# GATB/MindTheGap

Measured on AMD Instinct MI355X. Metric: breakpoints filled/sec, higher is better.
Workload: dtype u64; 1 GPU; synthetic human-scale: 3 Gbp i.i.d. donor as 600000 x 5 kb sequences, 100000 insertion sites (50-1000 nt) per batch, k=31, max-nodes 100; sites_per_batch=100000, sites_per_rank_and_step=100000, distinct_batches_per_rank=4, site_set=400000, donor_sequences=600000, erroneous_fragments=0, k=31, max_nodes=100, max_length=10000, nb_solid_kmers=3108581096, nb_unitigs=600024, index_bytes=60154587216, unitig_store_bytes=3945966160, batches_in_flight=6, input=prepared batches, resident in HBM, output=C-ABI records + ASCII sequences in page-locked host memory

## Files before the change

mindthegap_amd/csrc/mtg_emit.h:

```cpp
#ifndef MTG_EMIT_H
#define MTG_EMIT_H
#include "../../include/mtg_fill.h"
#include "mtg_copy.h"

namespace mtg {

enum : uint8_t { GAPF_REPEATED = 1, GAPF_REVERSE = 2 };

MTG_DEV void emit_plan(const GapOut& o, const PostOut& p, bool want_all, int k, uint32_t& nw, uint32_t& nc, uint32_t& asc, uint32_t& ext)
{
    nw = nc = asc = ext = 0;
    if (o.status != GAP_OK) return;
    if (want_all || (p.fast == 0 && p.nb_terminal > 0)) { nw = o.n_words; nc = o.n_contigs; }
    if (want_all) return;
    if (p.fast == 1) asc = p.pos - (uint32_t)k + 1u;
    else if (p.nb_terminal == 0 && o.n_contigs > 0 && p.clen0 > (uint32_t)k) ext = p.clen0 - (uint32_t)k + 1u;
}

struct PartTot {
    uint64_t begin[4], end[4];
    uint64_t lines, store_runs, run_nt, contig_nt, contig_words, post_lines, cov_kmers, copy_words, copy_cmds, cov_direct, n_lean;
    uint64_t copy_words_exec, copy_cmds_exec, scan_words;
    uint32_t n_retry, n_general, n_filled, n_ext;
    uint32_t n_parked, n_branching;
// ... 68 lines not shown
            U64x2 v;
            v.x = (uint64_t)out[0] | ((uint64_t)out[1] << 32);
            v.y = (uint64_t)out[2] | ((uint64_t)out[3] << 32);
            *reinterpret_cast<U64x2*>(d) = v;
        } else {
            for (uint32_t b = 0; b < n; b++) d[b] = (char)((out[b >> 2] >> (8u * (b & 3u))) & 0xFFu);
        }
    }
    if (lane == 0 && !(pk.half && aoff + L >= pk.x)) dst[L] = 0;
}
MTG_DEV void emit_ascii(const uint64_t* src, uint32_t from, uint32_t L, bool rc, char* dst) { emit_ascii_g<MTG_NLANES>(src, from, L, rc, dst, MTG_LANE()); }

struct EmitHost {
    char* seq;
    char* ext;
    mtg_filled* fil;
};
struct EmitDev {
    char* seq;
    char* ext;
    uint64_t seq_cap, ext_cap;
    mtg_gap_result* res;
    mtg_filled* fil;
    uint64_t* dense_words;
    uint32_t* dense_meta;
    uint64_t dense_cap_words, dense_cap_contigs;
    uint8_t* wire;
    uint64_t wire_cap, wire_tag;
    const PartTot* tot;
    uint32_t wire_gaps;
    uint32_t* shadow = nullptr;
    uint64_t shadow_cap = 0;
    uint32_t pack_q = 0;
};
MTG_DEV PackedTail packed_tail(const EmitDev& D) { return PackedTail{D.shadow, D.shadow ? packed_split(D.tot->end[2], D.pack_q) : 0ull, D.shadow_cap}; }
struct WireLayout {
    uint64_t o_gaps, o_filled, o_seq, o_ext, total;
};
MTG_HD WireLayout wire_layout(uint64_t n_gaps, uint64_t n_filled, uint64_t seq_bytes, uint64_t ext_bytes)
{
    WireLayout w;
    w.o_gaps = sizeof(mtg_wire_header);
    w.o_filled = w.o_gaps + ((n_gaps * sizeof(mtg_wire_gap) + 7) & ~7ull);
    w.o_seq = w.o_filled + ((n_filled * sizeof(mtg_wire_filled) + 7) & ~7ull);
    w.o_ext = w.o_seq + ((seq_bytes + 7) & ~7ull);
    w.total = w.o_ext + ((ext_bytes + 7) & ~7ull);
    return w;
}
MTG_HD uint64_t wire_word_sum(uint64_t w, uint64_t i) { return (w ^ (i * 0x9E3779B97F4A7C15ull)) * 0xBF58476D1CE4E5B9ull; }

MTG_DEV int qual_of(uint32_t errors, bool repeated)
{
    int q = repeated ? 25 : 50;
    if (errors == 1) q = 10;
    if (errors == 2) q = 5;
    return q;
}

MTG_DEV mtg_filled filled_of(const PostOut& p, uint64_t abase, uint32_t flags, const EmitHost& H)
{
    mtg_filled f;
    f.seq = H.seq + abase;
    f.nb_errors_in_anchor = (int)p.errors;
    f.target_index = (int)p.target;
#ifdef MTG_EMU
    f.avg_coverage = (float)p.ab_sum / (float)p.ab_n;
// ... 124 lines not shown
```

mindthegap_amd/csrc/mtg_gpu_fill.hip:

```cpp
#include "mtg_gpu_common.h"

namespace mtgi {

enum { TRAVERSAL_SETS = mtg_index::NWS };
__constant__ Index c_ix[TRAVERSAL_SETS];
__constant__ FillCfg c_cfg[TRAVERSAL_SETS];

#ifndef MTG_STAGE_A_WAVES
#define MTG_STAGE_A_WAVES 2
#endif
#ifndef MTG_WALK_WAVES
#define MTG_WALK_WAVES 2
#endif
enum { PARK_LISTS = 19 };
struct ParkCtl {
    uint32_t count[PARK_LISTS];
    uint32_t n_branching;
    uint32_t pad_[3];
#ifdef MTG_BUBBLE_TIMING
    uint32_t hist_lane[32], hist_wave[32], hist_walk_lane[32], hist_walk_wave[32];
#endif
};
#ifdef MTG_BUBBLE_TIMING
__device__ __forceinline__ void timing_note(uint32_t* hl, uint32_t* hw, uint64_t t0)
// ... 447 lines not shown
    for (uint32_t li = blockIdx.x; li < count; li += gridDim.x) {
    const uint32_t slot = use_list ? park_list(park, n, POST_LIST)[li] : li;
    __syncthreads();
    if (threadIdx.x == 0) {
        r = recs[slot];
        const ScanBlock& b = blocks[slot / SCAN_SL];
        r.wbase += b.v[0]; r.cbase += b.v[1]; r.abase += b.v[2]; r.ebase += b.v[3];
        r.rpos += (uint32_t)b.v[4]; r.gpos += (uint32_t)b.v[5]; r.fpos += (uint32_t)b.v[6];
        recs[slot] = r;
        if (r.o.status != GAP_OK) retry_list[r.rpos] = slot;
        else if (r.nc) general_list[r.gpos] = slot;
    }
    __syncthreads();
    GapScratch S;
    S.z = nullptr;
    S.v = nullptr;
    S.lane = slot & 63u;
    S.r = raw + (uint64_t)slot * cfg.raw_stride;
    S.h = head + (uint64_t)(slot >> 6) * cfg.hd_stride;
    const uint32_t g = ids ? ids[slot] : slot;
    emit_gap(us, cfg, S, r, gflags[g], slot, g, k, D, H);
    }
}
#ifndef MTG_EMIT_LEAN_G
#define MTG_EMIT_LEAN_G 8
#endif
enum { EMIT_LEAN_G = MTG_EMIT_LEAN_G };
__global__ void __launch_bounds__(64) k_emit_lean(UStore us, FillCfg cfg, uint8_t* raw, uint8_t* head, const SlotRec* __restrict__ recs, const ScanBlock* __restrict__ blocks, const uint32_t* __restrict__ ids,
                                                  const uint8_t* __restrict__ gflags, int k, EmitDev D, EmitHost H, uint32_t n)
{
    const uint32_t slot = blockIdx.x * (64u / EMIT_LEAN_G) + threadIdx.x / EMIT_LEAN_G, gl = threadIdx.x % EMIT_LEAN_G;
    if (slot >= n) return;
    const SlotRec r = recs[slot];
    if (!emit_is_lean(r, D)) return;
    GapScratch S;
    S.z = nullptr;
    S.v = nullptr;
    S.lane = slot & 63u;
    S.r = raw + (uint64_t)slot * cfg.raw_stride;
    S.h = head + (uint64_t)(slot >> 6) * cfg.hd_stride;
    const uint32_t g = ids ? ids[slot] : slot;
    emit_lean<EMIT_LEAN_G>(us, cfg, S, r, r.abase + blocks[slot / SCAN_SL].v[2], gflags[g], slot, g, k, D, H, gl);
}

__global__ void __launch_bounds__(256) k_wire_sum(uint8_t* wire, uint64_t cap)
{
    mtg_wire_header* h = reinterpret_cast<mtg_wire_header*>(wire);
    if (h->magic != 0x3145524957474D54ull || h->total_bytes > cap) return;
    const uint64_t* w = reinterpret_cast<const uint64_t*>(wire + sizeof(mtg_wire_header));
    const uint64_t n = (h->total_bytes - sizeof(mtg_wire_header)) / 8;
    uint64_t s = 0;
    for (uint64_t i = (uint64_t)blockIdx.x * blockDim.x + threadIdx.x; i < n; i += (uint64_t)gridDim.x * blockDim.x) s += wire_word_sum(w[i], i);
    for (int d = 32; d >= 1; d >>= 1) {
        const uint32_t lo = (uint32_t)__shfl_xor((int)(uint32_t)s, d, 64), hi = (uint32_t)__shfl_xor((int)(uint32_t)(s >> 32), d, 64);
        s += ((uint64_t)hi << 32) | lo;
    }
    if ((threadIdx.x & 63u) == 0 && s) atomicAdd(reinterpret_cast<unsigned long long*>(&h->checksum), (unsigned long long)s);
}

__global__ void __launch_bounds__(64) k_paths(FillCfg cfg, uint8_t* raw, uint8_t* head, const GapOut* __restrict__ outs, const uint32_t* __restrict__ slots, int k, uint32_t* out, uint32_t n)
{
    __shared__ PathsWork W;
    if (blockIdx.x >= n) return;
    const uint32_t slot = slots[blockIdx.x];
    GapScratch S;
    S.z = nullptr;
    S.v = nullptr;
    S.lane = slot & 63u;
    S.r = raw + (uint64_t)slot * cfg.raw_stride;
    S.h = head + (uint64_t)(slot >> 6) * cfg.hd_stride;
    paths_gap(cfg, S, outs[slot], k, W, out + (uint64_t)blockIdx.x * PATHS_WORDS);
}

__global__ void __launch_bounds__(64) k_general(Index ix, FillCfg cfg, uint8_t* raw, uint8_t* head, const GapOut* __restrict__ outs, const uint32_t* __restrict__ slots, const uint32_t* __restrict__ ids,
                                                const uint32_t* __restrict__ paths, const uint32_t* __restrict__ tcnt, const uint8_t* __restrict__ fast_ok, const uint64_t* __restrict__ src,
// ... 228 lines not shown
    uint64_t* d_tbad = d_tle + n_targets;
    uint32_t* d_pi_head = nullptr;
    uint32_t* d_pi_next = nullptr;
    uint32_t pi_mask = 0;
    uint8_t* d_tie_p = nullptr;
    if (seeds) {
        d_pi_head = const_cast<uint32_t*>(in.shared.pi);
        d_pi_next = d_pi_head + (size_t)in.shared.pi_mask + 1;
        pi_mask = in.shared.pi_mask;
        HIP_TRY(d_tie.alloc(n));
        d_tie_p = d_tie.as<uint8_t>();
        HIP_TRY(hipMemsetAsync(d_tie_p, 0, n, stream));
    } else if (n_targets >= (uint64_t)POST_INDEX_MIN * n && n_targets < (1ull << 30) && !tune::on(tune::T_NO_POST_INDEX)) {
        uint64_t cap = 1024;
        while (cap < 4 * n_targets) cap <<= 1;
        HIP_TRY(d_pidx.alloc((cap + 4 * n_targets) * 4));
        d_pi_head = d_pidx.as<uint32_t>();
        d_pi_next = d_pi_head + cap;
        pi_mask = (uint32_t)(cap - 1);
        HIP_TRY(hipMemsetAsync(d_pi_head, 0xFF, cap * 4, stream));
        hipLaunchKernelGGL(k_post_index, dim3((unsigned)std::min<size_t>(n, 4096)), dim3(256), 0, stream, d_pi_head, d_pi_next, pi_mask, (const uint64_t*)d_tle, (const uint64_t*)d_tbad, d_toff, d_tcnt, d_mis, (uint32_t)n, k);
        HIP_TRY(hipGetLastError());
    }
    HIP_TRY(d_tot.alloc(sizeof(PartTot)));
    uint64_t arena_used[2] = {0, 1};
    st.h2d_ms += now_ms() - t0;
    tick("upload (async)");

    const bool ktimers = tune::on(tune::T_KERNEL_TIMERS);
    hipEvent_t ev0, ev1 = nullptr, ev2, ev3, eve = nullptr, evc = nullptr, evf = nullptr, evl = nullptr, evl0 = nullptr;
    HIP_TRY(events.make(ev0));
    HIP_TRY(events.make(ev2));
    HIP_TRY(events.make(ev3));
    hipEvent_t evp;
    HIP_TRY(events.make(evp));
    if (ktimers) {
        HIP_TRY(events.make(eve));
        HIP_TRY(events.make(evc));
        HIP_TRY(events.make(ev1));
        HIP_TRY(events.make(evf));
        HIP_TRY(events.make(evl));
        HIP_TRY(events.make(evl0));
    }
    auto mark = [&](hipEvent_t e) -> hipError_t { return e ? hipEventRecord(e, stream) : hipSuccess; };
    PartTot* h_tot = (PartTot*)staging_host(&ws, Workspace::NHOST - 1, sizeof(PartTot) + 64);
    if (!h_tot) { set_error("no page-locked memory for the totals of a launch"); return MTG_ERR_NOMEM; }

    std::vector<uint32_t> todo;
    size_t n_todo = n;
    int rc = MTG_OK;
    const bool host_paths = tune::on(tune::T_HOST_PATHS);
    const bool want_records = sink.res != nullptr;
    size_t launches = 0;

    for (int tier = 0; tier <= MTG_MAX_TIER && n_todo; tier++) {
        FillCfg cfg = make_cfg(k, p->max_nodes, p->max_depth, p->end_rule_nonbranching, tier);
        const bool no_defer = tune::on(tune::T_NO_DEFER);
        if (no_defer || !idx->dev.us.nwords) cfg.cmd_cap = 0;
        const uint64_t per_gap = cfg.zero_stride + cfg.raw_stride + cfg.ilv_stride / 64 + cfg.hd_stride / 64 + sizeof(GapOut) + sizeof(SlotRec) + 64 + sizeof(mtg_gap_result) + sizeof(mtg_filled);
        const size_t cached = ws.cap[d_zero.slot] + ws.cap[d_raw.slot] + ws.cap[d_ilv.slot] + ws.cap[d_head.slot];
        size_t free_b = 0, total_b = 0;
        const uint64_t m0 = std::min<uint64_t>(n_todo, 1u << 20);
        const bool fits = ws.cap[d_zero.slot] >= m0 * cfg.zero_stride && ws.cap[d_raw.slot] >= m0 * cfg.raw_stride + 64 && ws.cap[d_ilv.slot] >= ((m0 + 63) / 64) * cfg.ilv_stride &&
                          ws.cap[d_head.slot] >= ((m0 + 63) / 64) * cfg.hd_stride;
        if (!fits) HIP_TRY(hipMemGetInfo(&free_b, &total_b));
        size_t chunk = fits ? (size_t)m0 : (size_t)(((double)free_b * 0.6 + (double)cached) / (double)per_gap);
        const size_t env_chunk = (size_t)tune::i(tune::T_MAX_CHUNK, 0);
        if (env_chunk && chunk > env_chunk) chunk = env_chunk;
// ... 111 lines not shown
#ifdef MTG_BUBBLE_TIMING
                {
                    static ParkCtl hc; static int shown = 0;
                    HIP_TRY(hipStreamSynchronize(stream));
                    HIP_TRY(hipMemcpy(&hc, d_park.p, sizeof hc, hipMemcpyDeviceToHost));
                    if (shown++ < 3) {
                        fprintf(stderr, "[timing] lists:"); for (int i = 0; i < PARK_LISTS; i++) fprintf(stderr, " %u", hc.count[i]); fprintf(stderr, "\n");
                        const char* nm[4] = {"bubble lane", "bubble wave", "resumed walk lane", "resumed walk wave"};
                        const uint32_t* hh[4] = {hc.hist_lane, hc.hist_wave, hc.hist_walk_lane, hc.hist_walk_wave};
                        for (int j = 0; j < 4; j++) { fprintf(stderr, "[timing] %s, log2(10 ns ticks) bins:", nm[j]); for (int i = 0; i < 24; i++) fprintf(stderr, " %u", hh[j][i]); fprintf(stderr, "\n"); }
                    }
                }
#endif
            }
            HIP_TRY(mark(ev1));
            HIP_TRY(mark(evl0));
            HIP_TRY(hipGetLastError());
            HIP_TRY(mark(evl));
            hipLaunchKernelGGL(k_copy, dim3((m + 3) / 4), dim3(256), 0, stream, idx->dev, cfg, d_raw.as<uint8_t>(), d_head.as<uint8_t>(), d_out.as<GapOut>(), park, m, (uint32_t)COPY_LIST);
            HIP_TRY(mark(evc));
            const uint32_t nblocks = (m + SCAN_SL - 1) / SCAN_SL;
            const uint32_t general_hint = ws.post_general == ~0u ? m : (uint32_t)std::min<uint64_t>(m, 4ull * ws.post_general + 1024ull);
            hipLaunchKernelGGL(k_post, dim3(general_hint), dim3(64), 0, stream, idx->dev, cfg, d_raw.as<uint8_t>(), d_head.as<uint8_t>(), d_out.as<GapOut>(), ids, d_tle, d_tbad, d_toff, d_tcnt, d_mis, d_fok,
                               in.want_all_contigs ? 1u : 0u, d_rec.as<SlotRec>(), m, park, (const uint32_t*)d_pi_head, (const uint32_t*)d_pi_next, pi_mask, d_rw, d_roff, d_tie_p);
            hipLaunchKernelGGL(k_post_lean, dim3((m + 64 / POST_LEAN_G - 1) / (64 / POST_LEAN_G)), dim3(64), 0, stream, idx->dev, cfg, d_raw.as<uint8_t>(), d_head.as<uint8_t>(), d_out.as<GapOut>(), in.want_all_contigs ? 1u : 0u, d_rec.as<SlotRec>(), m);
            const ScanBegin sbegin{{0, 0, arena_used[0], arena_used[1]}};
            hipLaunchKernelGGL(k_scan1, dim3(nblocks), dim3(SCAN_SL), 0, stream, d_rec.as<SlotRec>(), m, d_blocks.as<ScanBlock>());
            hipLaunchKernelGGL(k_scan2, dim3(1), dim3(256), 0, stream, d_blocks.as<ScanBlock>(), nblocks, sbegin, d_tot.as<PartTot>(), h_tot, park);
            HIP_TRY(hipGetLastError());
            EmitDev D;
            EmitHost H;
            const double share = std::min(1.0, std::max(0.0, tune::f(tune::T_PACKED_SEQ_SHARE, 0.0)));
            const uint32_t pack_q = (uint32_t)std::lround(share * 65536.0);
            bool packed = want_records && combo && identity && arena_used[0] == 0 && pack_q != 0;
            uint64_t shadow_halves = 0;
            if (packed) {
                shadow_halves = 2 * ((((uint64_t)sink.seq_cap * pack_q) >> 16) / 32 + 3);
                HIP_TRY(d_shadow.alloc(shadow_halves * 4));
            }
            auto emit = [&]() -> int {
                D.seq = sink.seq_dev ? sink.seq_dev : p_seq(); D.ext = d_ext.as<char>();
                D.seq_cap = sink.seq_cap; D.ext_cap = sink.ext_cap;
                D.res = p_res(); D.fil = p_fil();
                D.dense_words = d_dw.as<uint64_t>(); D.dense_meta = d_dm.as<uint32_t>();
                D.dense_cap_words = ws.cap[d_dw.slot] / 8; D.dense_cap_contigs = ws.cap[d_dm.slot] / 20;
                const bool want_wire = sink.wire_dev != nullptr && identity && tier == 0;
                D.wire = want_wire ? (uint8_t*)sink.wire_dev : nullptr; D.wire_cap = sink.wire_cap; D.wire_tag = sink.wire_tag;
                D.tot = d_tot.as<PartTot>(); D.wire_gaps = m;
                D.shadow = packed ? d_shadow.as<uint32_t>() : nullptr; D.shadow_cap = shadow_halves; D.pack_q = pack_q;
                if (packed) HIP_TRY(hipMemsetAsync(d_shadow.p, 0, shadow_halves * 4, stream));
                if (want_wire) HIP_TRY(hipMemsetAsync(sink.wire_dev, 0, sizeof(mtg_wire_header), stream));
                H.seq = sink.seq; H.ext = sink.ext; H.fil = sink.fil;
                if (!want_wire)
                    hipLaunchKernelGGL(k_emit_lean, dim3((m + 64 / EMIT_LEAN_G - 1) / (64 / EMIT_LEAN_G)), dim3(64), 0, stream, idx->dev.us, cfg, d_raw.as<uint8_t>(), d_head.as<uint8_t>(), d_rec.as<SlotRec>(), d_blocks.as<ScanBlock>(),
                                       ids, d_flags, k, D, H, m);
                hipLaunchKernelGGL(k_emit, dim3(want_wire ? m : general_hint), dim3(64), 0, stream, idx->dev.us, cfg, d_raw.as<uint8_t>(), d_head.as<uint8_t>(), d_rec.as<SlotRec>(), d_blocks.as<ScanBlock>(), ids, d_flags, k, D, H,
                                   d_rlist.as<uint32_t>(), d_glist.as<uint32_t>(), m, park, want_wire ? 0u : 1u);
                if (want_wire) hipLaunchKernelGGL(k_wire_sum, dim3(256 * 4), dim3(256), 0, stream, (uint8_t*)sink.wire_dev, sink.wire_cap);
                HIP_TRY(hipGetLastError());
                return MTG_OK;
            };
            HIP_TRY(mark(eve));
            if (int erc = emit()) return erc;
            HIP_TRY(hipEventRecord(ev2, stream));
            tick("host prep+launch");
            if (while_busy && !busy_done) { busy_done = true; (*while_busy)(); tick("host work during kernels"); }
            HIP_TRY(hipEventSynchronize(ev2));
            traversal_lock.unlock();
            tick("totals ready");
            t0 = now_ms();
            PartTot tot = *h_tot;
            const uint64_t need_w = tot.end[0] * 8 + 64, need_m = tot.end[1] * 20 + 64;
            bool again = false;
            if (want_records && tot.end[2] > sink.seq_cap) {
                const uintptr_t old = (uintptr_t)sink.seq, old_end = old + sink.seq_cap;
                const uintptr_t old_fil = (uintptr_t)sink.fil, old_fil_end = old_fil + n * sizeof(mtg_filled);
                if (!sink.grow_seq || !sink.grow_seq((size_t)tot.end[2], (size_t)tot.begin[2])) { set_error("sequence buffer too small: %llu bytes needed", (unsigned long long)tot.end[2]); return MTG_ERR_ARG; }
                if (launches > 1 && (uintptr_t)sink.seq != old)
                    for (size_t i = 0; i < n; i++) { const uintptr_t q = (uintptr_t)sink.fil[i].seq; if (q >= old && q < old_end) sink.fil[i].seq = sink.seq + (q - old); }
                if (launches > 1 && (uintptr_t)sink.fil != old_fil)
                    for (size_t i = 0; i < n; i++) { const uintptr_t q = (uintptr_t)sink.res[i].filled; if (q >= old_fil && q < old_fil_end) sink.res[i].filled = (const mtg_filled*)((const char*)sink.fil + (q - old_fil)); }
                again = true;
            }
            if (want_records && tot.end[3] > sink.ext_cap) {
                const uintptr_t old = (uintptr_t)sink.ext, old_end = old + sink.ext_cap;
                if (!sink.grow_ext || !sink.grow_ext((size_t)tot.end[3], (size_t)tot.begin[3])) { set_error("extension buffer too small: %llu bytes needed", (unsigned long long)tot.end[3]); return MTG_ERR_NOMEM; }
                if (launches > 1 && (uintptr_t)sink.ext != old)
                    for (size_t i = 0; i < n; i++) { const uintptr_t q = (uintptr_t)sink.res[i].extension; if (q >= old && q < old_end) sink.res[i].extension = sink.ext + (q - old); }
                again = true;
            }
            if (need_w > ws.cap[d_dw.slot] || need_m > ws.cap[d_dm.slot]) again = true;
            if (again) {
                HIP_TRY(hipStreamSynchronize(stream));
                if (combo) HIP_TRY(d_combo.grow_keeping(sink.combo_off_seq + std::max<size_t>(sink.seq_cap, 64) + SEQ_SLACK, sink.combo_off_seq + (size_t)tot.begin[2]));
                else if (!sink.seq_dev) HIP_TRY(d_seq.grow_keeping(std::max<size_t>(sink.seq_cap, 64) + SEQ_SLACK, (size_t)tot.begin[2]));
                HIP_TRY(d_ext.alloc(std::max<size_t>(sink.ext_cap, 64)));
                HIP_TRY(d_dw.alloc(need_w));
                HIP_TRY(d_dm.alloc(need_m));
                hipLaunchKernelGGL(k_scan1, dim3(nblocks), dim3(SCAN_SL), 0, stream, d_rec.as<SlotRec>(), m, d_blocks.as<ScanBlock>());
                hipLaunchKernelGGL(k_scan2, dim3(1), dim3(256), 0, stream, d_blocks.as<ScanBlock>(), nblocks, sbegin, d_tot.as<PartTot>(), (PartTot*)nullptr, park);
                packed = false;
                if (int erc = emit()) return erc;
            }
            CopyTurn copy_turn(idx->device);
            std::vector<mtg_gap_result> tmp_res;
            std::vector<mtg_filled> tmp_fil;
            const bool one_copy = combo && identity && tot.begin[2] == 0;
            const uint64_t pack_x = packed ? packed_split(tot.end[2], pack_q) : 0, pack_words = packed ? (tot.end[2] - pack_x + 31) / 32 : 0;
            uint64_t* h_shadow = nullptr;
            if (packed) {
                h_shadow = (uint64_t*)staging_host(&ws, Workspace::NHOST - 3, pack_words * 8 + 64);
                if (!h_shadow) { set_error("no page-locked memory for the packed sequences of a launch"); return MTG_ERR_NOMEM; }
            }
            if (want_records) {
                if (h_shadow) {
                    HIP_TRY(hipMemcpyAsync(sink.combo, d_combo.p, sink.combo_off_seq, hipMemcpyDeviceToHost, stream));
                    if (pack_words) HIP_TRY(hipMemcpyAsync(h_shadow, d_shadow.p, pack_words * 8, hipMemcpyDeviceToHost, stream));
                    HIP_TRY(hipEventRecord(evp, stream));
                    if (pack_x) HIP_TRY(hipMemcpyAsync(sink.combo + sink.combo_off_seq, (const char*)d_combo.p + sink.combo_off_seq, pack_x, hipMemcpyDeviceToHost, stream));
                } else if (one_copy) HIP_TRY(hipMemcpyAsync(sink.combo, d_combo.p, sink.combo_off_seq + (size_t)tot.end[2], hipMemcpyDeviceToHost, stream));
                else if (identity) {
                    HIP_TRY(hipMemcpyAsync(sink.res, p_res(), (size_t)m * sizeof(mtg_gap_result), hipMemcpyDeviceToHost, stream));
                    HIP_TRY(hipMemcpyAsync(sink.fil, p_fil(), (size_t)m * sizeof(mtg_filled), hipMemcpyDeviceToHost, stream));
                } else {
                    tmp_res.resize(m);
                    tmp_fil.resize(m);
                    HIP_TRY(hipMemcpyAsync(tmp_res.data(), p_res(), (size_t)m * sizeof(mtg_gap_result), hipMemcpyDeviceToHost, stream));
                    HIP_TRY(hipMemcpyAsync(tmp_fil.data(), p_fil(), (size_t)m * sizeof(mtg_filled), hipMemcpyDeviceToHost, stream));
                }
                const WireLayout wl = wire_layout(m, tot.n_filled, tot.end[2], tot.end[3]);
                const bool wired = sink.wire_dev != nullptr && identity && tier == 0 && wl.total <= sink.wire_cap && tot.n_retry == 0 && tot.n_general == 0;
                if (sink.wire_dev && identity && tier == 0) { sink.wire_ok = wired; sink.wire_bytes = wired ? wl.total : 0; }
                const char* seq_src = wired ? (const char*)sink.wire_dev + wl.o_seq : (sink.seq_dev ? sink.seq_dev : p_seq());
                if (!one_copy && !sink.seq_on_device && !sink.seq_stays_in_workspace && tot.end[2] > tot.begin[2]) HIP_TRY(hipMemcpyAsync(sink.seq + tot.begin[2], seq_src + tot.begin[2], tot.end[2] - tot.begin[2], hipMemcpyDeviceToHost, stream));
                if (tot.end[3] > tot.begin[3]) HIP_TRY(hipMemcpyAsync(sink.ext + tot.begin[3], d_ext.as<char>() + tot.begin[3], tot.end[3] - tot.begin[3], hipMemcpyDeviceToHost, stream));
            }
            std::vector<uint32_t> rlist(tot.n_retry), glist(tot.n_general);
            const bool dev_general = tot.n_general > 0 && !host_paths && !in.want_all_contigs && !tune::on(tune::T_HOST_GENERAL) && !tl_host_general;
            GenCtl* h_gctl = nullptr;
            GenDev GD{};
            if (dev_general) {
                const uint64_t ng = tot.n_general;
                HIP_TRY(d_paths.alloc(ng * (size_t)PATHS_WORDS * 4));
                HIP_TRY(d_ggaps.alloc(ng * sizeof(GenGap) + sizeof(GenCtl)));
                GD.cap_sols = 4 * ng + 1024; GD.cap_ascii = ng * 1280 + (1u << 20); GD.cap_tmp = ng * 48 + (1u << 17); GD.cap_bnd = 1u << 22;
                HIP_TRY(d_gsols.alloc(GD.cap_sols * sizeof(GenSol)));
                HIP_TRY(d_gascii.alloc(GD.cap_ascii + 64));
                HIP_TRY(d_gtmp.alloc(GD.cap_tmp * 8));
                HIP_TRY(d_gbnd.alloc(GD.cap_bnd * sizeof(NwCell)));
                GD.ctl = (GenCtl*)d_ggaps.p;
                GD.gaps = (GenGap*)((char*)d_ggaps.p + sizeof(GenCtl));
                GD.sols = d_gsols.as<GenSol>(); GD.ascii = d_gascii.as<char>(); GD.tmp = d_gtmp.as<uint64_t>(); GD.bnd = d_gbnd.as<NwCell>();
                HIP_TRY(hipMemsetAsync(GD.ctl, 0, sizeof(GenCtl), stream));
                hipLaunchKernelGGL(k_paths, dim3((unsigned)ng), dim3(64), 0, stream, cfg, d_raw.as<uint8_t>(), d_head.as<uint8_t>(), d_out.as<GapOut>(), d_glist.as<uint32_t>(), k, d_paths.as<uint32_t>(), (uint32_t)ng);
                hipLaunchKernelGGL(k_general, dim3((unsigned)ng), dim3(64), 0, stream, idx->dev, cfg, d_raw.as<uint8_t>(), d_head.as<uint8_t>(), d_out.as<GapOut>(), d_glist.as<uint32_t>(), ids, d_paths.as<uint32_t>(),
                                   d_tcnt, d_fok, d_src, d_flags, k, GD, (uint32_t)ng);
                HIP_TRY(hipGetLastError());
                h_gctl = (GenCtl*)staging_host(&ws, Workspace::NHOST - 2, sizeof(GenCtl) + ng * sizeof(GenGap) + 64);
                if (!h_gctl) { set_error("no page-locked memory for the multi-contig gaps of a launch"); return MTG_ERR_NOMEM; }
                HIP_TRY(hipMemcpyAsync(h_gctl, d_ggaps.p, sizeof(GenCtl) + ng * sizeof(GenGap), hipMemcpyDeviceToHost, stream));
            }
            HostChunk* hc = nullptr;
            SlotRec* h_rec = nullptr;
            uint64_t* h_w = nullptr;
            uint32_t* h_m = nullptr;
            const uint64_t tw = tot.end[0], tc = tot.end[1];
            if (tot.n_retry) HIP_TRY(hipMemcpyAsync(rlist.data(), d_rlist.p, (size_t)tot.n_retry * 4, hipMemcpyDeviceToHost, stream));
            auto contigs_to_host = [&]() -> int {
                hc->carve(m, tw, tc, h_rec, h_w, h_m);
                HIP_TRY(hipMemcpyAsync(h_rec, d_rec.p, (size_t)m * sizeof(SlotRec), hipMemcpyDeviceToHost, stream));
                if (tw) HIP_TRY(hipMemcpyAsync(h_w, d_dw.p, tw * 8, hipMemcpyDeviceToHost, stream));
                if (tc) HIP_TRY(hipMemcpyAsync(h_m, d_dm.p, tc * 20, hipMemcpyDeviceToHost, stream));
                return MTG_OK;
            };
            if (tot.n_general) {
                special.chunks.emplace_back(new HostChunk());
                hc = special.chunks.back().get();
                HIP_TRY(hipMemcpyAsync(glist.data(), d_glist.p, (size_t)tot.n_general * 4, hipMemcpyDeviceToHost, stream));
                if (!dev_general) { if (int crc = contigs_to_host()) return crc; }
            }
            HIP_TRY(hipEventRecord(ev3, stream));
            if (h_shadow) {
                HIP_TRY(hipEventSynchronize(evp));
                const double tx = now_ms();
                expand_packed_tail(h_shadow, sink.seq, pack_x, tot.end[2], sink.res, sink.fil, n, std::min(8, std::max(1, Pool::cpu_budget() / 2)));
                if (dbg) fprintf(stderr, "  [device_run] %-18s %.3f ms (%llu of %llu arena bytes from %llu words)\n", "packed tail", now_ms() - tx,
                                 (unsigned long long)(tot.end[2] - pack_x), (unsigned long long)tot.end[2], (unsigned long long)pack_words);
            }
            HIP_TRY(hipEventSynchronize(ev3));
            copy_turn.release();
            st.d2h_ms += now_ms() - t0;
            tick("results on the host");
            t0 = now_ms();
            st.index_lines += tot.lines; st.contig_nt += tot.contig_nt; st.store_runs += tot.store_runs; st.run_nt += tot.run_nt; st.post_lines += tot.post_lines;
            st.contig_words += tot.contig_words; st.coverage_kmers += tot.cov_kmers; st.dense_words += tw;
            st.copy_words += tot.copy_words; st.copy_cmds += tot.copy_cmds; st.coverage_direct_kmers += tot.cov_direct; st.n_lean_gaps += tot.n_lean;
            if (tier == 0 && identity) ws.post_general = m - (uint32_t)std::min<uint64_t>(tot.n_lean, m);
            st.copy_words_executed += tot.copy_words_exec; st.copy_cmds_executed += tot.copy_cmds_exec; st.post_scanned_words += tot.scan_words;
            sink.seq_used = tot.end[2];
            sink.ext_used = tot.end[3];
            arena_used[0] = tot.end[2];
            arena_used[1] = tot.end[3];
            sink.n_filled += tot.n_filled;
            if (want_records && !identity)
                for (uint32_t s2 = 0; s2 < m; s2++) { sink.res[host_ids[s2]] = tmp_res[s2]; sink.fil[host_ids[s2]] = tmp_fil[s2]; }
            for (uint32_t s2 : rlist) retry.push_back(host_ids ? host_ids[s2] : s2);
            if (tot.n_retry) sink.in_gap_order = false;
            if (hc && dev_general) {
                const uint64_t ng = tot.n_general;
                const GenCtl ctl = *h_gctl;
                const GenGap* hg = (const GenGap*)(h_gctl + 1);
                hc->gen_gaps.assign(hg, hg + ng);
                uint64_t n_host = 0;
                for (uint64_t i = 0; i < ng; i++) n_host += hg[i].status != GEN_OK;
                const uint64_t ns = std::min<uint64_t>(ctl.n_sols, GD.cap_sols), na = std::min<uint64_t>(ctl.ascii_bytes, GD.cap_ascii);
                hc->gen_sols.resize(ns);
                hc->gen_ascii.resize(na + 1);
                if (ns) HIP_TRY(hipMemcpyAsync(hc->gen_sols.data(), d_gsols.p, ns * sizeof(GenSol), hipMemcpyDeviceToHost, stream));
                if (na) HIP_TRY(hipMemcpyAsync(hc->gen_ascii.data(), d_gascii.p, na, hipMemcpyDeviceToHost, stream));
                if (host_ids) hc->gap_of.assign(host_ids, host_ids + m);
                const uint32_t chunk_id = (uint32_t)special.chunks.size() - 1;
                for (uint32_t i = 0; i < (uint32_t)ng; i++) special.special.push_back(SpecialGap{host_ids ? host_ids[glist[i]] : glist[i], chunk_id, glist[i], i});
                if (n_host) {
                    if (int crc = contigs_to_host()) return crc;
                    hc->path_of.assign(m, -1);
// ... 151 lines not shown
```

mindthegap_amd/csrc/mtg_host.cpp:

```cpp
#include "mtg_internal.h"
#include "mtg_dict_order.h"
#include <unistd.h>

#include <algorithm>
#include <atomic>
#include <chrono>
#include <cstdio>
#include <cstdlib>
#include <cstring>
#include <mutex>
#include <set>

extern "C" {
size_t mtg_tuning_count(void) { return (size_t)mtgi::tune::T_COUNT; }
int mtg_tuning_describe(size_t i, const char** name, const char** dflt, const char** kind, const char** what)
{
    using namespace mtgi::tune;
    if (i >= (size_t)T_COUNT) { mtgi::set_error("no tuning entry %zu", i); return MTG_ERR_ARG; }
    if (name) *name = g_entries[i].name;
    if (dflt) *dflt = g_entries[i].dflt;
    if (kind) *kind = g_entries[i].kind;
    if (what) *what = g_entries[i].what;
    return MTG_OK;
}
// ... 429 lines not shown
        char b[32] = {0};
        memcpy(b, s + i, n - i);
        const size_t r = n - i;
        out[w] = pack32(b) & (r < 32 ? (1ull << (2 * r)) - 1 : ~0ull);
    }
}
inline bool all_upper_acgt(const char* s, size_t n)
{
    static const struct Tab { bool ok[256]; Tab() { memset(ok, 0, sizeof ok); ok['A'] = ok['C'] = ok['G'] = ok['T'] = true; } } tab;
    bool ok = true;
    size_t i = 0;
#if defined(__x86_64__)
    static const bool vec = !tune::on(tune::T_NO_VEC);
    if (vec) {
        const __m128i A = _mm_set1_epi8('A'), C = _mm_set1_epi8('C'), G = _mm_set1_epi8('G'), T = _mm_set1_epi8('T');
        for (; i + 16 <= n; i += 16) {
            const __m128i v = _mm_loadu_si128(reinterpret_cast<const __m128i*>(s + i));
            const __m128i m = _mm_or_si128(_mm_or_si128(_mm_cmpeq_epi8(v, A), _mm_cmpeq_epi8(v, C)), _mm_or_si128(_mm_cmpeq_epi8(v, G), _mm_cmpeq_epi8(v, T)));
            if (_mm_movemask_epi8(m) != 0xFFFF) return false;
        }
    }
#endif
    for (; i < n; i++) ok &= tab.ok[(unsigned char)s[i]];
    return ok;
}
}

void expand_codes_scalar(const uint64_t* w, size_t b, size_t e, char* out)
{
    static const char NT[4] = {'A', 'C', 'T', 'G'};
    for (size_t i = b; i < e; i++) out[i] = NT[(w[i >> 5] >> (2 * (i & 31))) & 3];
}
#if defined(__x86_64__)
__attribute__((target("avx2"))) static void expand_codes_avx2(const uint64_t* w, size_t b, size_t e, char* out)
{
    size_t i = b;
    const size_t head = std::min(e, (b + 31) & ~(size_t)31);
    expand_codes_scalar(w, i, head, out);
    i = head;
    const __m256i spread = _mm256_setr_epi8(0, 0, 0, 0, 1, 1, 1, 1, 2, 2, 2, 2, 3, 3, 3, 3, 4, 4, 4, 4, 5, 5, 5, 5, 6, 6, 6, 6, 7, 7, 7, 7);
    const __m256i field = _mm256_set1_epi32((int)0xC0300C03u), low = _mm256_set1_epi8(0x0F);
    const __m256i lut = _mm256_setr_epi8('A', 'C', 'T', 'G', 'C', 0, 0, 0, 'T', 0, 0, 0, 'G', 0, 0, 0, 'A', 'C', 'T', 'G', 'C', 0, 0, 0, 'T', 0, 0, 0, 'G', 0, 0, 0);
    for (; i + 32 <= e; i += 32) {
        __m256i t = _mm256_and_si256(_mm256_shuffle_epi8(_mm256_set1_epi64x((long long)w[i >> 5]), spread), field);
        t = _mm256_and_si256(_mm256_or_si256(t, _mm256_srli_epi16(t, 4)), low);
        _mm256_storeu_si256(reinterpret_cast<__m256i*>(out + i), _mm256_shuffle_epi8(lut, t));
    }
    expand_codes_scalar(w, i, e, out);
}
static const bool have_avx2 = __builtin_cpu_supports("avx2") && !tune::on(tune::T_NO_VEC);
#endif
void expand_codes(const uint64_t* w, size_t b, size_t e, char* out)
{
#if defined(__x86_64__)
    if (have_avx2) { expand_codes_avx2(w, b, e, out); return; }
#endif
    expand_codes_scalar(w, b, e, out);
}

void expand_packed_tail(const uint64_t* w, char* seq, uint64_t x, uint64_t end, const mtg_gap_result* res, const mtg_filled* fil, size_t n, int nthreads)
{
    if (end <= x || n == 0) return;
    const size_t pieces = std::min<size_t>(n, 256);
    auto first_fill = [&](size_t g, size_t lim) { while (g < lim && res[g].n_filled == 0) g++; return g; };
    auto start_of = [&](size_t g) { return (uint64_t)(fil[g].seq - seq); };
    parallel_for(pieces, nthreads, [&](size_t c) {
        const size_t g0 = n * c / pieces, g1 = n * (c + 1) / pieces;
        const size_t f = first_fill(g0, g1);
        if (f == g1) return;
        const size_t nf = first_fill(g1, n);
        const uint64_t lo = std::max<uint64_t>(start_of(f), x), hi = std::min<uint64_t>(nf < n ? start_of(nf) : end, end);
        if (hi <= lo) return;
        expand_codes(w, lo - x, hi - x, seq + x);
        for (size_t g = f + 1; g < g1; g++) {
            if (res[g].n_filled == 0) continue;
            const uint64_t z = start_of(g) - 1;
            if (z >= lo && z < hi) seq[z] = 0;
        }
        seq[hi - 1] = 0;
    }, 1);
}

void FillInput::set_common(size_t g, std::string_view source, std::string_view swf_target, int nb_mis, uint8_t gap_flags)
{
    flags[g] = gap_flags;
    const uint64_t kfields = kmask(k);
    char sb[32] = {0};
    memcpy(sb, source.data(), (size_t)k);
    const uint64_t sp = pack32(sb) & kfields;
    src[g] = reverse_fields(sp) >> (64 - 2 * k);
    const size_t rl = swf_target.size(), w0 = roff[g];
    const size_t nw = (rl + 31) / 32 + 1;
    rwords[w0 + nw - 1] = 0;
    if (nw >= 2) rwords[w0 + nw - 2] = 0;
    pack_lsb(swf_target.data(), rl, rwords.p + w0);
    r0[g] = rl >= (size_t)k ? reverse_fields(rwords[w0] & kfields) >> (64 - 2 * k) : 0;
    if (!all_upper_acgt(swf_target.data(), rl)) { rlen[g] = 0xFFFFFFFFu; r0[g] = 0; }
    nbmis[g] = (uint8_t)nb_mis;
    bool ok = (int)source.size() == k;
    if (ok) {
        uint64_t c[4];
        memcpy(c, sb, 32);
        ok = ((c[0] | c[1] | c[2] | c[3]) & 0x0808080808080808ull) == 0;
    }
    fast_ok[g] = ok ? 1 : 0;
}
void FillInput::set_target(size_t o, std::string_view seq)
{
    uint8_t* slot = traw.p + o * TARGET_SLOT;
    const bool usable = (int)seq.size() >= k;
    memset(slot, 0, TARGET_SLOT);
    if (usable) memcpy(slot, seq.data(), (size_t)k);
    slot[TARGET_SLOT - 1] = usable ? 1 : 0;
// ... 1706 lines not shown
```

mindthegap_amd/csrc/mtg_internal.h:

```cpp
#ifndef MTG_INTERNAL_H
#define MTG_INTERNAL_H
#include "../../include/mtg_fill.h"
#include "mtg_hostutil.h"
#include "mtg_paths.h"
#include "mtg_general.h"
#include "mtg_emit.h"
#include "mtg_copy.h"
#include "mtg_format.h"
#include "mtg_tuning.h"
#include <algorithm>
#include <atomic>
#include <condition_variable>
#include <cstdio>
#include <cstdlib>
#include <cstring>
#include <functional>
#include <memory>
#include <mutex>
#include <sched.h>
#include <string>
#include <string_view>
#include <thread>
#include <vector>

// ... 185 lines not shown

template <typename G> inline uint64_t parallel_prefix(size_t n, int nthreads, uint64_t* out, G get)
{
    const size_t B = 4096, nb = (n + B - 1) / B;
    std::vector<uint64_t> bs(nb + 1, 0);
    out[0] = 0;
    parallel_for(nb, nthreads, [&](size_t b) {
        uint64_t sum = 0;
        for (size_t i = b * B; i < std::min(n, (b + 1) * B); i++) { const uint64_t v = get(i); out[i + 1] = v; sum += v; }
        bs[b + 1] = sum;
    }, 1);
    for (size_t b = 0; b < nb; b++) bs[b + 1] += bs[b];
    parallel_for(nb, nthreads, [&](size_t b) {
        uint64_t run = bs[b];
        for (size_t i = b * B; i < std::min(n, (b + 1) * B); i++) { run += out[i + 1]; out[i + 1] = run; }
    }, 1);
    return bs[nb];
}

struct Target {
    std::string_view seq, name;
    bool is_rc = false;
};
struct TargetSpan {
    const Target* p = nullptr;
    uint32_t n = 0;
    size_t size() const { return n; }
    const Target& operator[](size_t i) const { return p[i]; }
    const Target* begin() const { return p; }
    const Target* end() const { return p + n; }
};

void* staging_host(Workspace* ws, int slot, size_t bytes);
void expand_codes(const uint64_t* w, size_t b, size_t e, char* out);
void expand_codes_scalar(const uint64_t* w, size_t b, size_t e, char* out);
void expand_packed_tail(const uint64_t* w, char* seq, uint64_t x, uint64_t end, const mtg_gap_result* res, const mtg_filled* fil, size_t n, int nthreads);
void* pinned_alloc(size_t bytes);
void pinned_free(void* p);
int host_register(void* p, size_t bytes);
int host_unregister(void* p);
int device_download(const mtg_index* idx, void* host_dst, const void* dev_src, size_t bytes);
int device_upload(const mtg_index* idx, void* dev_dst, const void* host_src, size_t bytes);

template <typename T> struct Arr {
    T* p = nullptr;
    size_t n = 0;
    T* data() const { return p; }
    size_t size() const { return n; }
    bool empty() const { return n == 0; }
    T& operator[](size_t i) const { return p[i]; }
};
struct FillInput {
    int k = 31;
    bool want_all_contigs = false;
    Workspace* ws = nullptr;
    Arr<uint64_t> src;
    Arr<uint64_t> r0;
    Arr<uint32_t> roff;
    Arr<uint32_t> rlen;
    Arr<uint32_t> toff, tcnt;
    Arr<uint8_t> nbmis, fast_ok, flags;
    Arr<uint64_t> rwords;
    Arr<uint8_t> traw;
    void *block_a = nullptr, *block_b = nullptr, *block_c = nullptr;
    size_t bytes_a = 0, bytes_b = 0, bytes_c = 0;
    std::vector<uint64_t> own_a, own_b, own_c;
    void* dev_a = nullptr; void* dev_b = nullptr; void* dev_tenc = nullptr;
    bool text_mode = false;
// ... 331 lines not shown
```

Baseline: 224.4 million breakpoints/s.

## Emit per-slot sequence cursors on device and expand packed tail with streaming stores

The lean emit kernel now writes each slot's arena end offset into a cursor list placed ahead of the packed shadow buffer. The list comes back to the host in the same copy as the packed words. The host then expands the 2-bit tail into ASCII after the main event sync, instead of overlapping it with the remaining copies. Expansion runs single-threaded in 64 KB pieces, goes through a cache-resident buffer, and writes out with AVX2 non-temporal stores, replacing the multi-threaded per-gap scan of result records. In exchange, the expansion is serialized after the copies and loses thread parallelism, and the packed path is limited to sequence capacities that fit in 32 bits.

```diff
diff --git a/mindthegap_amd/csrc/mtg_emit.h b/mindthegap_amd/csrc/mtg_emit.h
--- a/mindthegap_amd/csrc/mtg_emit.h
+++ b/mindthegap_amd/csrc/mtg_emit.h
@@ -124,6 +124,7 @@
     uint32_t* shadow = nullptr;
     uint64_t shadow_cap = 0;
     uint32_t pack_q = 0;
+    uint32_t* cursor = nullptr;
 };
 MTG_DEV PackedTail packed_tail(const EmitDev& D) { return PackedTail{D.shadow, D.shadow ? packed_split(D.tot->end[2], D.pack_q) : 0ull, D.shadow_cap}; }
 struct WireLayout {
diff --git a/mindthegap_amd/csrc/mtg_gpu_fill.hip b/mindthegap_amd/csrc/mtg_gpu_fill.hip
--- a/mindthegap_amd/csrc/mtg_gpu_fill.hip
+++ b/mindthegap_amd/csrc/mtg_gpu_fill.hip
@@ -503,6 +503,8 @@
     const uint32_t slot = blockIdx.x * (64u / EMIT_LEAN_G) + threadIdx.x / EMIT_LEAN_G, gl = threadIdx.x % EMIT_LEAN_G;
     if (slot >= n) return;
     const SlotRec r = recs[slot];
+    const uint64_t abase = r.abase + blocks[slot / SCAN_SL].v[2];
+    if (D.cursor && gl == 0) D.cursor[slot] = (uint32_t)(abase + r.asc);
     if (!emit_is_lean(r, D)) return;
     GapScratch S;
     S.z = nullptr;
@@ -511,7 +513,7 @@
     S.r = raw + (uint64_t)slot * cfg.raw_stride;
     S.h = head + (uint64_t)(slot >> 6) * cfg.hd_stride;
     const uint32_t g = ids ? ids[slot] : slot;
-    emit_lean<EMIT_LEAN_G>(us, cfg, S, r, r.abase + blocks[slot / SCAN_SL].v[2], gflags[g], slot, g, k, D, H, gl);
+    emit_lean<EMIT_LEAN_G>(us, cfg, S, r, abase, gflags[g], slot, g, k, D, H, gl);
 }
 
 __global__ void __launch_bounds__(256) k_wire_sum(uint8_t* wire, uint64_t cap)
@@ -806,8 +808,6 @@
     HIP_TRY(events.make(ev0));
     HIP_TRY(events.make(ev2));
     HIP_TRY(events.make(ev3));
-    hipEvent_t evp;
-    HIP_TRY(events.make(evp));
     if (ktimers) {
         HIP_TRY(events.make(eve));
         HIP_TRY(events.make(evc));
@@ -985,11 +985,12 @@
             EmitHost H;
             const double share = std::min(1.0, std::max(0.0, tune::f(tune::T_PACKED_SEQ_SHARE, 0.0)));
             const uint32_t pack_q = (uint32_t)std::lround(share * 65536.0);
-            bool packed = want_records && combo && identity && arena_used[0] == 0 && pack_q != 0;
+            bool packed = want_records && combo && identity && arena_used[0] == 0 && pack_q != 0 && sink.seq_cap <= 0xFFFFFFFFull;
             uint64_t shadow_halves = 0;
+            const size_t list_bytes = packed ? ((size_t)m * 4 + 63) & ~(size_t)63 : 0;
             if (packed) {
                 shadow_halves = 2 * ((((uint64_t)sink.seq_cap * pack_q) >> 16) / 32 + 3);
-                HIP_TRY(d_shadow.alloc(shadow_halves * 4));
+                HIP_TRY(d_shadow.alloc(list_bytes + shadow_halves * 4));
             }
             auto emit = [&]() -> int {
                 D.seq = sink.seq_dev ? sink.seq_dev : p_seq(); D.ext = d_ext.as<char>();
@@ -1000,8 +1001,9 @@
                 const bool want_wire = sink.wire_dev != nullptr && identity && tier == 0;
                 D.wire = want_wire ? (uint8_t*)sink.wire_dev : nullptr; D.wire_cap = sink.wire_cap; D.wire_tag = sink.wire_tag;
                 D.tot = d_tot.as<PartTot>(); D.wire_gaps = m;
-                D.shadow = packed ? d_shadow.as<uint32_t>() : nullptr; D.shadow_cap = shadow_halves; D.pack_q = pack_q;
-                if (packed) HIP_TRY(hipMemsetAsync(d_shadow.p, 0, shadow_halves * 4, stream));
+                D.cursor = packed ? d_shadow.as<uint32_t>() : nullptr;
+                D.shadow = packed ? (uint32_t*)(d_shadow.as<char>() + list_bytes) : nullptr; D.shadow_cap = shadow_halves; D.pack_q = pack_q;
+                if (packed) HIP_TRY(hipMemsetAsync(D.shadow, 0, shadow_halves * 4, stream));
                 if (want_wire) HIP_TRY(hipMemsetAsync(sink.wire_dev, 0, sizeof(mtg_wire_header), stream));
                 H.seq = sink.seq; H.ext = sink.ext; H.fil = sink.fil;
                 if (!want_wire)
@@ -1056,20 +1058,22 @@
                 if (int erc = emit()) return erc;
             }
             CopyTurn copy_turn(idx->device);
+            tick("link turn");
             std::vector<mtg_gap_result> tmp_res;
             std::vector<mtg_filled> tmp_fil;
             const bool one_copy = combo && identity && tot.begin[2] == 0;
             const uint64_t pack_x = packed ? packed_split(tot.end[2], pack_q) : 0, pack_words = packed ? (tot.end[2] - pack_x + 31) / 32 : 0;
+            uint32_t* h_cursor = nullptr;
             uint64_t* h_shadow = nullptr;
             if (packed) {
-                h_shadow = (uint64_t*)staging_host(&ws, Workspace::NHOST - 3, pack_words * 8 + 64);
-                if (!h_shadow) { set_error("no page-locked memory for the packed sequences of a launch"); return MTG_ERR_NOMEM; }
+                h_cursor = (uint32_t*)staging_host(&ws, Workspace::NHOST - 3, list_bytes + pack_words * 8 + 64);
+                if (!h_cursor) { set_error("no page-locked memory for the packed sequences of a launch"); return MTG_ERR_NOMEM; }
+                h_shadow = (uint64_t*)((char*)h_cursor + list_bytes);
             }
             if (want_records) {
                 if (h_shadow) {
                     HIP_TRY(hipMemcpyAsync(sink.combo, d_combo.p, sink.combo_off_seq, hipMemcpyDeviceToHost, stream));
-                    if (pack_words) HIP_TRY(hipMemcpyAsync(h_shadow, d_shadow.p, pack_words * 8, hipMemcpyDeviceToHost, stream));
-                    HIP_TRY(hipEventRecord(evp, stream));
+                    HIP_TRY(hipMemcpyAsync(h_cursor, d_shadow.p, list_bytes + pack_words * 8, hipMemcpyDeviceToHost, stream));
                     if (pack_x) HIP_TRY(hipMemcpyAsync(sink.combo + sink.combo_off_seq, (const char*)d_combo.p + sink.combo_off_seq, pack_x, hipMemcpyDeviceToHost, stream));
                 } else if (one_copy) HIP_TRY(hipMemcpyAsync(sink.combo, d_combo.p, sink.combo_off_seq + (size_t)tot.end[2], hipMemcpyDeviceToHost, stream));
                 else if (identity) {
@@ -1133,17 +1137,19 @@
                 if (!dev_general) { if (int crc = contigs_to_host()) return crc; }
             }
             HIP_TRY(hipEventRecord(ev3, stream));
-            if (h_shadow) {
-                HIP_TRY(hipEventSynchronize(evp));
-                const double tx = now_ms();
-                expand_packed_tail(h_shadow, sink.seq, pack_x, tot.end[2], sink.res, sink.fil, n, std::min(8, std::max(1, Pool::cpu_budget() / 2)));
-                if (dbg) fprintf(stderr, "  [device_run] %-18s %.3f ms (%llu of %llu arena bytes from %llu words)\n", "packed tail", now_ms() - tx,
-                                 (unsigned long long)(tot.end[2] - pack_x), (unsigned long long)tot.end[2], (unsigned long long)pack_words);
-            }
             HIP_TRY(hipEventSynchronize(ev3));
             copy_turn.release();
+            tick("results on the host");
+            if (h_shadow) {
+                expand_packed_list(h_shadow, sink.seq, pack_x, tot.end[2], h_cursor, m);
+                if (dbg) {
+                    const double t = now_ms();
+                    fprintf(stderr, "  [device_run] %-18s %.3f ms (%llu of %llu arena bytes from %llu words)\n", "packed tail", t - tk,
+                            (unsigned long long)(tot.end[2] - pack_x), (unsigned long long)tot.end[2], (unsigned long long)pack_words);
+                    tk = t;
+                }
+            }
             st.d2h_ms += now_ms() - t0;
-            tick("results on the host");
             t0 = now_ms();
             st.index_lines += tot.lines; st.contig_nt += tot.contig_nt; st.store_runs += tot.store_runs; st.run_nt += tot.run_nt; st.post_lines += tot.post_lines;
             st.contig_words += tot.contig_words; st.coverage_kmers += tot.cov_kmers; st.dense_words += tw;
diff --git a/mindthegap_amd/csrc/mtg_host.cpp b/mindthegap_amd/csrc/mtg_host.cpp
--- a/mindthegap_amd/csrc/mtg_host.cpp
+++ b/mindthegap_amd/csrc/mtg_host.cpp
@@ -485,21 +485,38 @@
     for (size_t i = b; i < e; i++) out[i] = NT[(w[i >> 5] >> (2 * (i & 31))) & 3];
 }
 #if defined(__x86_64__)
+__attribute__((target("avx2"))) static inline __m256i letters32(uint64_t word)
+{
+    const __m256i spread = _mm256_setr_epi8(0, 0, 0, 0, 1, 1, 1, 1, 2, 2, 2, 2, 3, 3, 3, 3, 4, 4, 4, 4, 5, 5, 5, 5, 6, 6, 6, 6, 7, 7, 7, 7);
+    const __m256i field = _mm256_set1_epi32((int)0xC0300C03u), low = _mm256_set1_epi8(0x0F);
+    const __m256i lut = _mm256_setr_epi8('A', 'C', 'T', 'G', 'C', 0, 0, 0, 'T', 0, 0, 0, 'G', 0, 0, 0, 'A', 'C', 'T', 'G', 'C', 0, 0, 0, 'T', 0, 0, 0, 'G', 0, 0, 0);
+    __m256i t = _mm256_and_si256(_mm256_shuffle_epi8(_mm256_set1_epi64x((long long)word), spread), field);
+    t = _mm256_and_si256(_mm256_or_si256(t, _mm256_srli_epi16(t, 4)), low);
+    return _mm256_shuffle_epi8(lut, t);
+}
 __attribute__((target("avx2"))) static void expand_codes_avx2(const uint64_t* w, size_t b, size_t e, char* out)
 {
     size_t i = b;
     const size_t head = std::min(e, (b + 31) & ~(size_t)31);
     expand_codes_scalar(w, i, head, out);
     i = head;
-    const __m256i spread = _mm256_setr_epi8(0, 0, 0, 0, 1, 1, 1, 1, 2, 2, 2, 2, 3, 3, 3, 3, 4, 4, 4, 4, 5, 5, 5, 5, 6, 6, 6, 6, 7, 7, 7, 7);
-    const __m256i field = _mm256_set1_epi32((int)0xC0300C03u), low = _mm256_set1_epi8(0x0F);
-    const __m256i lut = _mm256_setr_epi8('A', 'C', 'T', 'G', 'C', 0, 0, 0, 'T', 0, 0, 0, 'G', 0, 0, 0, 'A', 'C', 'T', 'G', 'C', 0, 0, 0, 'T', 0, 0, 0, 'G', 0, 0, 0);
-    for (; i + 32 <= e; i += 32) {
-        __m256i t = _mm256_and_si256(_mm256_shuffle_epi8(_mm256_set1_epi64x((long long)w[i >> 5]), spread), field);
-        t = _mm256_and_si256(_mm256_or_si256(t, _mm256_srli_epi16(t, 4)), low);
-        _mm256_storeu_si256(reinterpret_cast<__m256i*>(out + i), _mm256_shuffle_epi8(lut, t));
-    }
+    for (; i + 32 <= e; i += 32) _mm256_storeu_si256(reinterpret_cast<__m256i*>(out + i), letters32(w[i >> 5]));
     expand_codes_scalar(w, i, e, out);
+}
+__attribute__((target("avx2"))) static void expand_range_streaming(const uint64_t* w, char* seq, uint64_t x, const uint32_t* c, const uint32_t* ce, uint64_t lo, uint64_t hi)
+{
+    alignas(64) char buf[8192];
+    for (uint64_t b = lo; b < hi; b += sizeof buf) {
+        const uint64_t e = std::min<uint64_t>(b + sizeof buf, hi);
+        const size_t nb = (size_t)(e - b);
+        const uint64_t* wb = w + ((b - x) >> 5);
+        for (size_t j = 0; 32 * j < nb; j++) _mm256_store_si256(reinterpret_cast<__m256i*>(buf + 32 * j), letters32(wb[j]));
+        for (; c < ce && *c <= e; c++) buf[*c - 1 - b] = 0;
+        size_t i = 0;
+        for (; i + 32 <= nb; i += 32) _mm256_stream_si256(reinterpret_cast<__m256i*>(seq + b + i), _mm256_load_si256(reinterpret_cast<const __m256i*>(buf + i)));
+        memcpy(seq + b + i, buf + i, nb - i);
+    }
+    _mm_sfence();
 }
 static const bool have_avx2 = __builtin_cpu_supports("avx2") && !tune::on(tune::T_NO_VEC);
 #endif
@@ -511,27 +528,32 @@
     expand_codes_scalar(w, b, e, out);
 }
 
-void expand_packed_tail(const uint64_t* w, char* seq, uint64_t x, uint64_t end, const mtg_gap_result* res, const mtg_filled* fil, size_t n, int nthreads)
+void expand_packed_range(const uint64_t* w, char* seq, uint64_t x, const uint32_t* cursor, size_t n, uint64_t lo, uint64_t hi)
+{
+    const uint32_t* c = std::upper_bound(cursor, cursor + n, (uint32_t)lo), * const ce = cursor + n;
+#if defined(__x86_64__)
+    if (have_avx2 && ((uintptr_t)(seq + lo) & 31) == 0) { expand_range_streaming(w, seq, x, c, ce, lo, hi); return; }
+#endif
+    expand_codes(w, lo - x, hi - x, seq + x);
+    for (; c < ce && *c <= hi; c++) seq[*c - 1] = 0;
+}
+void expand_packed_list(const uint64_t* w, char* seq, uint64_t x, uint64_t end, const uint32_t* cursor, size_t n, size_t piece)
+{
+    if (end <= x) return;
+    for (uint64_t lo = x; lo < end; lo += piece) expand_packed_range(w, seq, x, cursor, n, lo, std::min<uint64_t>(lo + piece, end));
+    seq[end - 1] = 0;
+}
+
+void expand_packed_tail(const uint64_t* w, char* seq, uint64_t x, uint64_t end, const mtg_gap_result* res, const mtg_filled* fil, size_t n, int)
 {
     if (end <= x || n == 0) return;
-    const size_t pieces = std::min<size_t>(n, 256);
-    auto first_fill = [&](size_t g, size_t lim) { while (g < lim && res[g].n_filled == 0) g++; return g; };
-    auto start_of = [&](size_t g) { return (uint64_t)(fil[g].seq - seq); };
-    parallel_for(pieces, nthreads, [&](size_t c) {
-        const size_t g0 = n * c / pieces, g1 = n * (c + 1) / pieces;
-        const size_t f = first_fill(g0, g1);
-        if (f == g1) return;
-        const size_t nf = first_fill(g1, n);
-        const uint64_t lo = std::max<uint64_t>(start_of(f), x), hi = std::min<uint64_t>(nf < n ? start_of(nf) : end, end);
-        if (hi <= lo) return;
-        expand_codes(w, lo - x, hi - x, seq + x);
-        for (size_t g = f + 1; g < g1; g++) {
-            if (res[g].n_filled == 0) continue;
-            const uint64_t z = start_of(g) - 1;
-            if (z >= lo && z < hi) seq[z] = 0;
-        }
-        seq[hi - 1] = 0;
-    }, 1);
+    std::vector<uint32_t> cursor(n);
+    uint64_t next = end;
+    for (size_t g = n; g-- > 0;) {
+        cursor[g] = (uint32_t)next;
+        if (res[g].n_filled) next = (uint64_t)(fil[g].seq - seq);
+    }
+    expand_packed_list(w, seq, x, end, cursor.data(), n);
 }
 
 void FillInput::set_common(size_t g, std::string_view source, std::string_view swf_target, int nb_mis, uint8_t gap_flags)
diff --git a/mindthegap_amd/csrc/mtg_internal.h b/mindthegap_amd/csrc/mtg_internal.h
--- a/mindthegap_amd/csrc/mtg_internal.h
+++ b/mindthegap_amd/csrc/mtg_internal.h
@@ -241,8 +241,11 @@
 };
 
 void* staging_host(Workspace* ws, int slot, size_t bytes);
+enum : size_t { EXPAND_PIECE = 65536 };
 void expand_codes(const uint64_t* w, size_t b, size_t e, char* out);
 void expand_codes_scalar(const uint64_t* w, size_t b, size_t e, char* out);
+void expand_packed_range(const uint64_t* w, char* seq, uint64_t x, const uint32_t* cursor, size_t n, uint64_t lo, uint64_t hi);
+void expand_packed_list(const uint64_t* w, char* seq, uint64_t x, uint64_t end, const uint32_t* cursor, size_t n, size_t piece = EXPAND_PIECE);
 void expand_packed_tail(const uint64_t* w, char* seq, uint64_t x, uint64_t end, const mtg_gap_result* res, const mtg_filled* fil, size_t n, int nthreads);
 void* pinned_alloc(size_t bytes);
 void pinned_free(void* p);
```

Result: slower. 190.3 million breakpoints/s (-15.2%).
